# shendurelab/MIPGEN

Hardware: AMD Instinct MI355X
Metric: candidate MIPs scored/sec (SVR) (higher is better)
Workload: dtype f64

## Files before the change

mipgen_amd/csrc/accel_tiles.hip:

```cpp
#include "accel_internal.h"

extern "C" {

int mipgen_pick_sv_split(int n_tiles, int n_sv, int n_cu)
{
    const int groups = (n_sv + SVR_GROUP - 1) / SVR_GROUP;
    const double PH0 = 6.0;
    int best = 1;
    double best_cost = 0;
    for (int s = 1; s <= 8; s++) {
        if (s > 1 && groups / s < 32) break;
        const int64_t units = (int64_t)n_tiles * s, rounds = (units + n_cu - 1) / n_cu;
        const double cost = (double)rounds * (PH0 + (double)((groups + s - 1) / s));
        if (s == 1 || cost < best_cost * 0.98) { best = s; best_cost = cost; }
    }
    return best;
}

int mipgen_ensure_events(mipgen_accel* h)
{
    const size_t want = 4 * h->windows.size();
    while (h->ev.size() < want) {
        hipEvent_t e = nullptr;
        HIP_TRY(hipEventCreate(&e));
// ... 96 lines not shown
    auto shape_of = [&](const DevRegion& d, bool few) -> const Shape& {
        const int lanes = 64 * (few ? h->geom_few.wpc : h->geom.wpc);
        const uint64_t key = ((uint64_t)(uint32_t)d.n_pos << 32) | ((uint64_t)(uint16_t)d.k0 << 16) | (uint64_t)(uint16_t)d.n_sizes | (few ? (uint64_t)1 << 15 : 0);
        auto it = shapes.find(key);
        if (it != shapes.end()) return it->second;
        Shape best;
        double best_cost = 0;
        const int Cmax = D.max_capture - d.k0 * D.inc;
        for (int kc_cap = std::min(9, d.n_sizes); kc_cap >= 1; kc_cap--) {
            const int nkc = (d.n_sizes + kc_cap - 1) / kc_cap;
            if (kc_cap < std::min(9, d.n_sizes) && nkc == (d.n_sizes + kc_cap) / (kc_cap + 1)) continue;
            std::vector<Run> runs;
            double ent = 0, slots = 0;
            size_t lds_r = 0;
            bool ok = true;
            for (int c = 0; c < nkc && ok; c++) {
                const int ki0 = (int)((int64_t)d.n_sizes * c / nkc), ki1 = (int)((int64_t)d.n_sizes * (c + 1) / nkc);
                const int kc = ki1 - ki0;
                const int Cmax_t = Cmax - ki0 * D.inc, Cmin_t = Cmax_t - (kc - 1) * D.inc;
                const int ssmax = Cmax_t - D.min_sum, ssmin = Cmin_t - D.max_sum, ssr = ssmax - ssmin + 1;
                int np = std::max(1, std::min(lanes / kc, d.n_pos));
                size_t lds_t = 0;
                for (; np >= 1; np--) {
                    lds_t = mipgen_svr_lds_bytes_tile(np, ssr, ssmax, Lmax, n_arm, h->geom.group, h->geom.n_e, h->geom.n_l, h->geom.nchunk * h->geom.wpc * 64);
                    if (lds_t <= 160 * 1024) break;
                }
                if (np < 1) { ok = false; break; }
                { const int np_cf = np - ((np + D.inc) % 32); if (np_cf >= 1 && np_cf * 10 >= np * 9) { np = np_cf; lds_t = mipgen_svr_lds_bytes_tile(np, ssr, ssmax, Lmax, n_arm, h->geom.group, h->geom.n_e, h->geom.n_l, h->geom.nchunk * h->geom.wpc * 64); } }
                { const int nt = (d.n_pos + np - 1) / np, np_even = (d.n_pos + nt - 1) / nt;
                  if (np_even < np) { np = np_even; lds_t = mipgen_svr_lds_bytes_tile(np, ssr, ssmax, Lmax, n_arm, h->geom.group, h->geom.n_e, h->geom.n_l, h->geom.nchunk * h->geom.wpc * 64); } }
                runs.push_back({ki0, kc, np});
                lds_r = std::max(lds_r, lds_t);
                const double tiles = std::ceil((double)d.n_pos / np);
                ent += tiles * (np * (h->geom.n_e + h->geom.n_l) / 2.0 + (np + ssr - 1) * (h->geom.n_e + h->geom.n_l) / 2.0 + (double)np * ssr);
                slots += tiles * lanes;
            }
            if (!ok) continue;
            const double cost = 47.0 * ent + 2.7 * slots * D.n_pairs / 1.0;
            if (best.runs.empty() || cost < best_cost) { best.runs = runs; best_cost = cost; best.lds = lds_r; }
        }
        return shapes.emplace(key, std::move(best)).first->second;
    };
    for (Window& w : h->windows) {
        w.svr_tile0 = (int)st.size();
        int n_few_regions = 0;
        for (int i = w.r0; i < w.r1; i++) if (h->hregions[i].n_pos > 0 && h->hregions[i].n_sizes == 1) n_few_regions++;
        const bool win_few = h->have_few && n_few_regions >= h->n_cu;
        std::vector<uint8_t> st_few;
        for (int i = w.r0; i < w.r1; i++) {
            const DevRegion& d = h->hregions[i];
            if (d.n_pos <= 0 || d.n_sizes <= 0) continue;
            const bool few = win_few && d.n_sizes == 1;
            const Shape& shape = shape_of(d, false);
            if (shape.runs.empty()) { svr_lds = (size_t)1 << 30; continue; }
            svr_lds = std::max(svr_lds, shape.lds);
            const int Cmax = D.max_capture - d.k0 * D.inc;
            for (size_t lvl = 0; lvl < shape.runs.size(); lvl++) {
                const Run& r = shape.runs[lvl];
                max_levels = std::max(max_levels, (int)lvl + 1);
                for (int p0 = 0; p0 < d.n_pos; p0 += r.np) {
                    const int npt = std::min(r.np, d.n_pos - p0);
                    const int Cmax_t = Cmax - r.ki0 * D.inc, ssmax = Cmax_t - D.min_sum, ssr = (r.kc - 1) * D.inc + D.max_sum - D.min_sum + 1;
                    const double ent = (npt + (npt + ssr - 1)) * (h->geom.n_e + h->geom.n_l) / 2.0 + (double)npt * ssr;
                    const double cost = 19.0 * ent + 100.0 * (npt + ssmax + 2 * Lmax) + 75000.0;
                    const int fits = mipgen_svr_scores_fit_lds(npt, r.kc, D.n_pairs, ssr, ssmax, Lmax, n_arm, h->geom.group, h->geom.n_e, h->geom.n_l, h->geom.nchunk * h->geom.wpc * 64);
                    for (int s2 = 0; s2 < 2; s2++) { SvrTile t = {i, s2, p0, npt, r.ki0, r.kc, (int)lvl, fits}; st.push_back(t); st_cost.push_back(cost); st_few.push_back(few ? 1 : 0); }
                }
            }
        }
        {
            const size_t t0 = (size_t)w.svr_tile0, n = st.size() - t0;
            std::vector<size_t> order(n);
            for (size_t k = 0; k < n; k++) order[k] = k;
            std::stable_sort(order.begin(), order.end(), [&](size_t a, size_t b) { return st_few[a] != st_few[b] ? st_few[a] < st_few[b] : st_cost[t0 + a] > st_cost[t0 + b]; });
            std::vector<SvrTile> sorted(n);
            for (size_t k = 0; k < n; k++) sorted[k] = st[t0 + order[k]];
            std::copy(sorted.begin(), sorted.end(), st.begin() + (ptrdiff_t)t0);
            w.n_svr_few = 0;
            for (size_t k = 0; k < n; k++) w.n_svr_few += st_few[k];
        }
        w.n_svr_tiles = (int)st.size() - w.svr_tile0;
        {
            const size_t t0 = (size_t)w.svr_tile0, n = (size_t)w.n_svr_tiles;
            int wl = 0;
            for (size_t k = 0; k < n; k++) wl = std::max(wl, st[t0 + k].level + 1);
            w.lvl_tile0.assign(1, (int)st_lvl.size());
            for (int lvl = 0; lvl < wl; lvl++) {
                for (size_t k = 0; k < n; k++) if (st[t0 + k].level == lvl) st_lvl.push_back(st[t0 + k]);
                w.lvl_tile0.push_back((int)st_lvl.size());
// ... 35 lines not shown
```

mipgen_amd/csrc/common.h:

```cpp
#pragma once
#include <stdint.h>
#include "../../include/mipgen_accel.h"

#define BASE_A 0
#define BASE_C 1
#define BASE_G 2
#define BASE_T 3
#define BASE_N 4
#define BASE_DASH 5
#define BASE_OTHER 6
#define BASE_CODE_MASK 7
#define BASE_MASKED_BIT 8
#define BASE_SNP_SHIFT 4

#define F_EXT 0
#define F_EXT_GC 15
#define F_EXT_LEN 21
#define F_LRC 22
#define F_INS 66
#define F_INS_GC 129
#define F_INS_LEN 151
#define F_LIG 152
#define F_LIG_GC 167
#define F_LIG_LEN 173
// ... 91 lines not shown
    const int32_t* order;
};

struct SvrGeom {
    int32_t nchunk;
    int32_t chunk_len;
    int32_t n_e, n_l;
    int32_t group;
    int32_t wpc;
    int32_t pad[2];
};

#define SVR_MAX_CHUNK 15
#define SVR_GROUP 3
#define SVR_MAX_THREADS 1024
#define LOG_THREADS 256

#define SVR_N_ARR 7
struct SvrLayout {
    int rinv, lg10, rows, pf, tb, it;
    int ku, kd, ci, pf_stride;
    int tj, ti;
    int tu, td, tb_stride;
    int ssr_p;
    int bytes_kpar;
    int bytes_desc, bytes_ent, bytes_idx, bytes_sb, bytes_psum;
    int n_ent;
    int n_ent_lds;
    int total_bytes;
    int nq, ins_len, up_cnt, dn_cnt, span_b, rinv_len;
    int ins_sl, up_sl, dn_sl;
};

#if defined(__HIPCC__)
__host__ __device__
#endif
__attribute__((always_inline)) static inline int svr_arr_len(const SvrLayout& L, int k) { return k < 3 ? +L.ins_len : (k < 5 ? +L.up_cnt : +L.dn_cnt); }
#if defined(__HIPCC__)
__host__ __device__
#endif
__attribute__((always_inline)) static inline int svr_pad_slots(int len) { return (((len + 1 + 15) / 16) | 1) * 16; }
#if defined(__HIPCC__)
__host__ __device__
#endif
__attribute__((always_inline)) static inline int svr_arr_off(const SvrLayout& L, int k)
{
    const int ki = k < 3 ? k : 3, ku = k < 3 ? 0 : (k < 5 ? k - 3 : 2), kd = k < 5 ? 0 : k - 5;
    return ki * L.ins_sl + ku * L.up_sl + kd * L.dn_sl;
}
#if defined(__HIPCC__)
__host__ __device__
#endif
__attribute__((always_inline)) static inline int svr_arr_chunk(const SvrLayout& L, int k) { return (k < 3 ? +L.ins_sl : (k < 5 ? +L.up_sl : +L.dn_sl)) / 16; }
#if defined(__HIPCC__)
__host__ __device__
#endif
__attribute__((always_inline)) static inline SvrLayout svr_layout(int np, int ssmin, int ssmax, int Lmax, int n_arm, int group, int n_up, int n_dn, int n_threads)
{
    SvrLayout L;
    const int ssr = ssmax - ssmin + 1;
    L.nq = np + ssr - 1;
    L.ins_len = np + ssmax;
    L.up_cnt = Lmax + np;
    L.dn_cnt = L.nq + Lmax;
    L.ins_sl = svr_pad_slots(L.ins_len); L.up_sl = svr_pad_slots(L.up_cnt); L.dn_sl = svr_pad_slots(L.dn_cnt);
    L.span_b = np + ssmax + 2 * Lmax + 1;
    L.rinv_len = (ssmax > Lmax ? ssmax : Lmax) + 2;
    int o = 0;
    L.rinv = o; o += 3 * L.rinv_len;
    L.lg10 = o; o += 102 + 44;
    L.n_ent = np * n_up + L.nq * n_dn;
    L.rows = o; o += 2 * group * SV_ROW;
    int g = 3 * L.ins_sl + 2 * L.up_sl + 2 * L.dn_sl;
    L.ku = g; g += n_arm; L.kd = g; g += n_arm;
    L.ci = g; g += 1;
    L.tj = g; g += 18;
    L.ti = g; g += ssr;
    L.pf_stride = g;
    int pf_doubles = 2 * group * L.pf_stride;
    const int scratch_doubles = (np * (80 * 4 + ssr * 16) + 7) / 8;
    if (pf_doubles < scratch_doubles) pf_doubles = scratch_doubles;
    L.pf = o; o += pf_doubles;
    L.tu = 0; L.td = np * n_arm; L.tb_stride = np * n_arm + L.nq * n_arm;
    L.tb = o; o += group * L.tb_stride;
    L.ssr_p = ssr | 1;
    L.it = o; o += group * np * L.ssr_p;
    int bytes = o * 8;
    L.bytes_desc = bytes; bytes += SVR_N_ARR * 16 * 4;
    L.n_ent_lds = L.n_ent; (void)n_threads;
    L.bytes_ent = bytes; bytes += 2 * L.n_ent_lds * 4;
    L.bytes_psum = bytes; bytes += 2 * SVR_MAX_CHUNK * (SVR_MAX_THREADS / 64) + 16;
    bytes = (bytes + 15) & ~15;
    L.bytes_kpar = bytes; bytes += 64;
    L.bytes_idx = bytes;
    bytes += 4 * (3 * L.ins_sl + 2 * L.up_sl + 2 * L.dn_sl);
    L.bytes_sb = bytes; bytes += L.span_b + 8;
    L.total_bytes = (bytes + 15) & ~15;
    return L;
}
```

mipgen_amd/csrc/kernels.h:

```cpp
#pragma once
#include <hip/hip_runtime.h>
#include "common.h"
#include "reads_common.h"
#include "call_model.h"

struct HostConsts;
struct LrcMers { int8_t k[MIPGEN_N_LRC], code[MIPGEN_N_LRC], rc[MIPGEN_N_LRC]; };
struct FmtRegion {
    int32_t chr_off, chr_len;
    int32_t label_off, label_len;
    int32_t feature_start, feature_stop;
    int64_t rb0;
};
struct FmtConst {
    char middle[96];
    int32_t middle_len;
    int32_t n_regions;
    int64_t first_index;
};

struct KmerParams {
    int32_t n_k;
    int32_t k[MIPGEN_MAX_OLIGO];
    int32_t kmax;
// ... 17 lines not shown
    const uint2* __restrict__ units;
    int64_t n_small, n_big;
    const uint32_t* __restrict__ start;
    const int32_t* __restrict__ mol_len;
    const int64_t* __restrict__ pos_off;
    int32_t n;
    int64_t n_pos;
    uint32_t cell0;
    int min_family, min_quality;
};

struct CallCounters { unsigned long long tested, too_deep, candidates, calls; };
#define MIPGEN_CALL_MAX_POSITIONS (((int64_t)1 << 29) - 1)

struct LocusCounters { unsigned long long covered, bases, discordant, deletions, insertions, ins_discordant; };

extern "C" {
size_t mipgen_logistic_lds_bytes(int span);
hipError_t mipgen_launch_records_logistic(hipStream_t, int score, int n_tiles, int span_max, const DevParams*, const DevRegion*, const LogTile*, const uint8_t*, const int32_t*,
                                          const uint8_t*, const HostConsts*, double*, uint64_t*, int64_t* sat_idx, unsigned int* sat_count, unsigned int sat_cap);
size_t mipgen_logistic_dense_lds_bytes(int np_all, int np, int ssr, int ssmax, int Lmax, int n_up, int n_dn);
hipError_t mipgen_launch_logistic_dense(hipStream_t, int n_tiles, size_t lds_bytes, const DevParams*, const DevRegion*, const SvrTile*, const uint8_t*, const int32_t*,
                                        const uint8_t*, const HostConsts*, double*, uint64_t*, int64_t* sat_idx, unsigned int* sat_count, unsigned int sat_cap);
size_t mipgen_svr_lds_bytes_tile(int np, int ss_range, int ssmax, int Lmax, int n_arm, int group, int n_e, int n_l, int n_threads);
int mipgen_svr_scores_fit_lds(int np, int kc, int n_pairs, int ss_range, int ssmax, int Lmax, int n_arm, int group, int n_e, int n_l, int n_threads);
hipError_t mipgen_launch_svr_dense(hipStream_t, int n_tiles, int n_tiles_few, size_t lds_bytes, const DevParams*, const SvrGeom*, const SvrGeom* geom_few, const DevRegion*,
                                   const SvrTile*, const uint8_t*, const int32_t*, const double* log10_tab, const double* model, int n_sv, double gamma_l2e, double rho,
                                   double s_guard, const uint64_t* records, double* scores, int64_t n_cand, int n_split, double* partials);
hipError_t mipgen_launch_svr_run_state(hipStream_t s, int64_t n_pos, const DevParams* P, const DevRegion* regions, const int32_t* pos_region, const int32_t* pos_local,
                                       const uint32_t* run_bounds, int max_levels, int level, double margin, const double* scores, const uint64_t* records, double* pbs,
                                       uint8_t* state);
hipError_t mipgen_launch_svr_tile_keep(hipStream_t s, int n_tiles, const SvrTile* tiles, const int64_t* region_pos0, int64_t win_pos0, const uint8_t* state, int64_t* keep);
hipError_t mipgen_launch_svr_tile_compact(hipStream_t s, int n_tiles, const SvrTile* tiles, const int64_t* keep, const int64_t* offs, SvrTile* out, const DevParams* P,
                                          const DevRegion* regions, double* scores, unsigned long long* skipped);
hipError_t mipgen_launch_svr_gemm(hipStream_t, int n, const double* feats, const uint64_t* records, const double* model_t, const double* sv_norm, const double* sv_coef,
                                  const double* center, int n_sv_pad, double gamma, double rho, double* scores);
hipError_t mipgen_launch_dense_candidates(hipStream_t, const DevParams* P, const DevRegion* regions, int r0, int r1, int64_t c0, int n, mipgen_candidate* out);
hipError_t mipgen_launch_dense_list_fix(hipStream_t, int n, const uint64_t* records, double rho, double s_guard, double* scores);
hipError_t mipgen_launch_features_batch(hipStream_t, int n, const DevParams*, const DevRegion*, const mipgen_candidate*, const uint8_t* bases, const int32_t* copy,
                                        const uint8_t* unmap, const HostConsts*, uint64_t* records, double* features);
hipError_t mipgen_launch_candidates(hipStream_t, int n, const DevParams*, const DevRegion*, const mipgen_candidate*, const uint8_t*, const int32_t*, const uint8_t*,
                                    const HostConsts*, const double* model, int n_sv, double gamma, double rho, int method, double*, uint64_t*, double*, mipgen_candidate_ints*,
                                    int literal, const unsigned int* n_dev);
hipError_t mipgen_launch_candidates_probes(hipStream_t, int n, const ProbeSrc*, const HostConsts*, const double* model, int n_sv, double gamma, double rho, int method,
                                           double*, uint64_t*, double*, mipgen_candidate_ints*, int literal, const unsigned int* n_dev);
hipError_t mipgen_launch_probe_features(hipStream_t, int n, const ProbeSrc*, const HostConsts*, uint64_t* records, double* features);
hipError_t mipgen_launch_print_boundary_scan(hipStream_t, const DevParams*, const DevRegion*, const RescoreSrc*, double tol_rel, double tol_abs, mipgen_candidate* out,
                                             int64_t* out_idx, unsigned int* count, unsigned int cap, int n_cu);
// ... 82 lines not shown
```

mipgen_amd/csrc/kernels_svr.hip:

```cpp
#include <hip/hip_runtime.h>
#include "kernels.h"
#include "device_utils.h"
#include "exp2_coef.h"
#include "mip_record.h"
#include <stdlib.h>

namespace {

__device__ __forceinline__ void exp2x3(double& t0, double& t1, double& t2)
{
    constexpr double C[11] = EXP2_COEF_10;
    const double MAGIC = 6755399441055744.0;
    double m0, m1, m2, f0, f1, f2;
    const double cd = C[10];
    asm volatile(
        "v_add_f64 %[m0], %[t0], %[magic]\n\t"
        "v_add_f64 %[m1], %[t1], %[magic]\n\t"
        "v_add_f64 %[m2], %[t2], %[magic]\n\t"
        "v_add_f64 %[f0], %[m0], -%[magic]\n\t"
        "v_add_f64 %[f1], %[m1], -%[magic]\n\t"
        "v_add_f64 %[f2], %[m2], -%[magic]\n\t"
        "v_add_f64 %[f0], %[t0], -%[f0]\n\t"
        "v_add_f64 %[f1], %[t1], -%[f1]\n\t"
        "v_add_f64 %[f2], %[t2], -%[f2]\n\t"
// ... 33 lines not shown
          [c5] "s"(C[5]), [c6] "s"(C[6]), [c7] "s"(C[7]), [c8] "s"(C[8]), [c9] "s"(C[9]));
    t0 = __hiloint2double(__double2hiint(t0) + (__double2loint(m0) << 20), __double2loint(t0));
    t1 = __hiloint2double(__double2hiint(t1) + (__double2loint(m1) << 20), __double2loint(t1));
    t2 = __hiloint2double(__double2hiint(t2) + (__double2loint(m2) << 20), __double2loint(t2));
}

template <int N>
__device__ __forceinline__ double dpp_row_shr(double x)
{
    const int lo = __builtin_amdgcn_update_dpp(0, __double2loint(x), 0x110 | N, 0xf, 0xf, true);
    const int hi = __builtin_amdgcn_update_dpp(0, __double2hiint(x), 0x110 | N, 0xf, 0xf, true);
    return __hiloint2double(hi, lo);
}
__device__ __forceinline__ double readlane_f64(double x, int l)
{
    return __hiloint2double(__builtin_amdgcn_readlane(__double2hiint(x), l), __builtin_amdgcn_readlane(__double2loint(x), l));
}

__device__ __forceinline__ int arm_feat(int base, int idx) { return base + idx + (idx >= 15); }
__device__ __forceinline__ int ins_feat(int idx) { return F_INS + idx + (idx >= 63); }

}

extern "C" int mipgen_svr_scores_fit_lds(int np, int kc, int n_pairs, int ss_range, int ssmax, int Lmax, int n_arm, int group, int n_e, int n_l, int n_threads)
{
    const SvrLayout La = svr_layout(np, ssmax - ss_range + 1, ssmax, Lmax, n_arm, group, n_e, n_l, n_threads);
    const SvrLayout Lb = svr_layout(np, ssmax - ss_range + 1, ssmax, Lmax, n_arm, group, n_l, n_e, n_threads);
    const int need = np * kc * n_pairs;
    return need <= La.total_bytes / 8 - La.pf && need <= Lb.total_bytes / 8 - Lb.pf;
}

extern "C" size_t mipgen_svr_lds_bytes_tile(int np, int ss_range, int ssmax, int Lmax, int n_arm, int group, int n_e, int n_l, int n_threads)
{
    const SvrLayout La = svr_layout(np, ssmax - ss_range + 1, ssmax, Lmax, n_arm, group, n_e, n_l, n_threads);
    const SvrLayout Lb = svr_layout(np, ssmax - ss_range + 1, ssmax, Lmax, n_arm, group, n_l, n_e, n_threads);
    if ((size_t)La.tb_stride * group * 8 > 65535 || (size_t)Lb.tb_stride * group * 8 > 65535) return (size_t)1 << 30;
    const size_t a = (size_t)La.total_bytes, b = (size_t)Lb.total_bytes;
    return a > b ? a : b;
}

__device__ __forceinline__ void svr_steps2(double& a0, double& a1, uint32_t lu, uint32_t ld, uint32_t pg0, uint32_t pg1,
                                           double i00, double i01, double i02, double i10, double i11, double i12)
{
    double u00, u01, u02, d00, d01, d02, u10, u11, u12, d10, d11, d12;
    uint32_t au0, ad0, au1, ad1, s0, s1, s2, s3;
    asm volatile(
        "s_and_b32 %[s0], %[pg0], 0xffff\n\t"
        "s_lshr_b32 %[s1], %[pg0], 16\n\t"
        "s_and_b32 %[s2], %[pg1], 0xffff\n\t"
        "s_lshr_b32 %[s3], %[pg1], 16\n\t"
        "v_add_u32 %[au0], %[s0], %[lu]\n\t"
        "v_add_u32 %[ad0], %[s1], %[ld]\n\t"
        "v_add_u32 %[au1], %[s2], %[lu]\n\t"
        "v_add_u32 %[ad1], %[s3], %[ld]\n\t"
        "ds_read_b64 %[u00], %[au0]\n\t"
        "ds_read_b64 %[d00], %[ad0]\n\t"
        "ds_read_b64 %[u01], %[au0] offset:8\n\t"
        "ds_read_b64 %[d01], %[ad0] offset:8\n\t"
// ... 134 lines not shown
    const double* __restrict__ model = model_all + (int64_t)sv0 * SV_ROW;
    const int n_sv = max(0, min(n_sv_all - sv0, gpp * SVR_GROUP));
    const int tid = threadIdx.x, lane = tid & (WAVE - 1);
    const int wid = __builtin_amdgcn_readfirstlane(tid / WAVE);
    const int NT = blockDim.x, NW = NT / WAVE;
    const bool minus = tile.strand != 0;

    const int A = P->n_pairs;
    const int Lmax = max(P->e_max, P->l_max);
    const int n_arm = max(G.n_e, G.n_l) | 1;
    const int Cmax_t = P->max_capture - (R.k0 + tile.ki0) * P->inc;
    const int Cmin_t = Cmax_t - (tile.kc - 1) * P->inc;
    const int ssmax = Cmax_t - P->min_sum, ssmin = Cmin_t - P->max_sum;
    const int p_first = R.first_pos + tile.p0;
    const int lo = p_first - Lmax;
    const int up_min = minus ? +P->l_min : +P->e_min;
    const int dn_min = minus ? +P->e_min : +P->l_min;
    const int n_up = minus ? +G.n_l : +G.n_e, n_dn = minus ? +G.n_e : +G.n_l;
    const int up_base = minus ? F_LIG : F_EXT, dn_base = minus ? F_EXT : F_LIG;
    const int up_len_f = minus ? F_LIG_LEN : F_EXT_LEN, dn_len_f = minus ? F_EXT_LEN : F_LIG_LEN;
    const int up_cp_f = minus ? F_LLC : F_LEC, dn_cp_f = minus ? F_LEC : F_LLC;
    const int up_norm_f = minus ? SVR_N_LIG : SVR_N_EXT, dn_norm_f = minus ? SVR_N_EXT : SVR_N_LIG;

    const SvrLayout L = svr_layout(tile.np, ssmin, ssmax, Lmax, n_arm, SVR_GROUP, n_up, n_dn, (int)blockDim.x);
    int L_ku = L.ku, L_kd = L.kd, L_tu = L.tu, L_td = L.td, L_ins = L.ins_len, L_up = L.up_cnt, L_dn = L.dn_cnt;
    asm volatile("" : "+s"(L_ku), "+s"(L_kd), "+s"(L_tu), "+s"(L_td), "+s"(L_ins), "+s"(L_up), "+s"(L_dn));
    const int S_ins = __builtin_amdgcn_readfirstlane(L.ins_sl), S_up = __builtin_amdgcn_readfirstlane(L.up_sl), S_dn = __builtin_amdgcn_readfirstlane(L.dn_sl);
    double* const dbase = (double*)smem;
    double* rinv = dbase + L.rinv;
    double* lg10 = dbase + L.lg10;
    uint32_t* ent_a = (uint32_t*)(smem + L.bytes_ent);
    uint32_t* ent_b = ent_a + L.n_ent_lds;
    const double cneg = -gamma_l2e, c2 = 2.0 * gamma_l2e;
    uint16_t* psum = (uint16_t*)(smem + L.bytes_psum);
    uint32_t* work = (uint32_t*)(smem + L.bytes_psum + 2 * SVR_MAX_CHUNK * (SVR_MAX_THREADS / 64));
    double* rows = dbase + L.rows;
    double* pfb = dbase + L.pf;
    double* tbb = dbase + L.tb;
    double* itb = dbase + L.it;
    ScanDesc* desc = (ScanDesc*)(smem + L.bytes_desc);
    uint32_t* sidx = (uint32_t*)(smem + L.bytes_idx);
    uint8_t* sb = smem + L.bytes_sb;
    const int ssr = ssmax - ssmin + 1;
    const int nq_t = L.nq;

    for (int i = tid; i < L.span_b + 8; i += NT) {
        int ri = lo + i - R.seq_start;
        sb[i] = (i < L.span_b && ri >= 0 && ri < R.seq_len) ? (bases[R.seq_off + ri] & BASE_CODE_MASK) : (uint8_t)BASE_OTHER;
    }
    for (int i = tid; i < L.rinv_len; i += NT) {
        rinv[3 * i] = i > 0 ? 1.0 / (double)i : 0.0; rinv[3 * i + 1] = i > 1 ? 1.0 / (double)(i - 1) : 0.0;
        rinv[3 * i + 2] = i > 2 ? 1.0 / (double)(i - 2) : 0.0;
    }
    for (int i = tid; i < 102; i += NT) lg10[i] = i == 0 ? 0.0 : (i <= 100 ? log10_tab[i] : 2.0);
    for (int i = tid; i < MIPGEN_N_LRC; i += NT) lg10[102 + i] = R.lrc[i];
    for (int i = tid; i < A && i < SVR_MAX_CHUNK * (SVR_MAX_THREADS / 64); i += NT) psum[i] = (uint16_t)(P->arm_ext[i] + P->arm_lig[i]);
    if (tid < SVR_N_ARR) {
        ScanDesc d;
        const int k = tid;
        const bool ins = k < 3, up = k == 3 || k == 4;
        d.o0 = ins ? Lmax : (up ? 0 : Lmax + ssmin);
        d.k = ins ? k + 1 : ((k - 3) & 1) + 1;
        d.ax = ins ? 21 : 5; d.ay = ins ? 5 : 1; d.thr = ins ? 63 : 15;
        d.base = ins ? F_INS : (up ? up_base : dn_base);
        d.len = ins ? L_ins : (up ? L_up : L_dn);
        d.out = (ins ? k : 3) * S_ins + (ins ? 0 : (up ? k - 3 : 2)) * S_up + (k < 5 ? 0 : k - 5) * S_dn;
        d.ixo = d.out; d.c = (ins ? +S_ins : (up ? +S_up : +S_dn)) / 16;
        d.blk = ins ? 1 : ((up ? minus : !minus) ? 2 : 0);
        desc[k] = d;
    }
    __syncthreads();

    for (int k = 0; k < SVR_N_ARR; k++) {
        const ScanDesc d = desc[k];
        for (int i = tid; i < 16 * d.c; i += NT) {
            int slot = SVR_ZERO;
            if (i < d.len) {
                const int b0 = sb[d.o0 + i], b1 = sb[d.o0 + i + 1], b2 = sb[d.o0 + i + 2];
                const int last = d.k == 1 ? b0 : (d.k == 2 ? b1 : b2);
// ... 19 lines not shown
        (void)norm;
        int cp = 1;
        if (R.copy_off >= 0) {
            const int slot = P->len_slot[len];
            const int ri = lo + s - R.seq_start;
            cp = (slot >= 0 && ri >= 0 && ri < R.seq_len) ? copy[R.copy_off + (int64_t)slot * R.seq_len + ri] : 0;
        }
        const uint32_t cpc = (uint32_t)min(max(cp, 0), 101);
        uint32_t jcode = 0;
        if (is_lig) {
            int j0, j1;
            if (!minus) { j0 = sb[s]; j1 = sb[s + 1]; }
            else { j0 = comp_code(sb[s + len - 1]); j1 = comp_code(sb[s + len - 2]); }
            jcode = (j0 < 4 && j1 < 4) ? (uint32_t)(4 * j0 + j1 + 1) : 17u;
        }
        const int s0 = up ? s : wl;
        e_a = (uint32_t)((3 * S_ins + (up ? 0 : 2 * S_up) + s0) * (SVR_GROUP * 8)) | ((uint32_t)(((up ? L_tu : L_td) + wl * n_arm + li) * (SVR_GROUP * 8)) << 16);
        e_b = (uint32_t)len | ((uint32_t)up << 7) | ((jcode * (SVR_GROUP * 8)) << 8) | ((cpc * 8) << 17);
    };
    for (int w = tid; w < n_ent; w += NT) { uint32_t ea_, eb_; arm_entry(w, ea_, eb_, nullptr); ent_a[w] = ea_; ent_b[w] = eb_; }

    const int chunk = wid / G.wpc;
    const int item = (wid - chunk * G.wpc) * WAVE + lane;
    int np_lane = tile.np + (32 - (tile.np + P->inc) % 32) % 32;
    if (np_lane * tile.kc > G.wpc * WAVE) np_lane = tile.np;
    const int kci_l = item / np_lane, pl_l = item - kci_l * np_lane;
    const bool owner = chunk < G.nchunk && kci_l < tile.kc && pl_l < tile.np;
    const int kci = owner ? kci_l : 0, pl = owner ? pl_l : 0;
    const int a_lo = min(chunk, G.nchunk - 1) * G.chunk_len;
    const int a_n = min(G.chunk_len, A - a_lo);
    const int C = Cmax_t - kci * P->inc;
    const uint32_t lane_u_off = (uint32_t)((L.tu + pl * n_arm) * (SVR_GROUP * 8));
    const uint32_t lane_d_off = (uint32_t)((L.td + (pl + C - P->max_sum - ssmin) * n_arm) * (SVR_GROUP * 8));
    const int prog0 = __builtin_amdgcn_readfirstlane((minus ? MIPGEN_MAX_ARM_PAIRS + 16 : 0) + a_lo);
    uint32_t newS_v = 0;
#pragma unroll
    for (int i = 0; i < CL; i++) {
        const int a = a_lo + min(i, a_n - 1);
        if (i == 0 || (i < a_n && P->arm_ext[a - 1] + P->arm_lig[a - 1] != P->arm_ext[a] + P->arm_lig[a])) newS_v |= 1u << i;
    }
    const uint32_t newS = __builtin_amdgcn_readfirstlane(newS_v);
    const int iB = (pl * L.ssr_p + (C - ssmin)) * SVR_GROUP;
    double acc[CL];
#pragma unroll
    for (int i = 0; i < CL; i++) acc[i] = 0.0;
    const bool wave_owns = __builtin_amdgcn_ballot_w64(owner) != 0;

    if (tid == 0) {
        int* kp = (int*)(smem + L.bytes_kpar);
        kp[0] = nU; kp[1] = n_up; kp[2] = n_dn; kp[3] = up_min; kp[4] = dn_min; kp[5] = Lmax; kp[6] = ssmin; kp[7] = n_ent;
        kp[8] = L_tu; kp[9] = L_td; kp[10] = n_arm; kp[11] = tile.np; kp[12] = ssmax; kp[13] = L.ssr_p; kp[14] = minus ? 1 : 0;
    }

    const int n_groups = (n_sv + SVR_GROUP - 1) / SVR_GROUP;
    constexpr int ROW_N = SVR_GROUP * SV_ROW;
    constexpr int ROW_R = 1;
    const int64_t row_lim = (int64_t)n_sv * SV_ROW;
    auto row_fetch = [&](int k, int j) -> double {
        const int64_t gk = (int64_t)k * ROW_N + j;
        return (j < ROW_N && gk < row_lim) ? model[gk] : 0.0;
    };
    auto row_slot = [&](int k, int j) -> int { const int g = j / SV_ROW; return (k & 1) * ROW_N + (j - g * SV_ROW) * SVR_GROUP + g; };
    auto load_rows_direct = [&](int k) __attribute__((always_inline)) { for (int j = tid; j < ROW_N; j += NT) rows[row_slot(k, j)] = row_fetch(k, j); };

    typedef __attribute__((address_space(3))) const double lds_cd;
    typedef volatile __attribute__((address_space(3))) const double lds_vcd;
    typedef __attribute__((address_space(3))) double lds_d;
    typedef __attribute__((address_space(3))) const uint32_t lds_cu;
    constexpr int S_UNITS = 7;
    auto stage_scan = [&](int k) __attribute__((always_inline)) {
        lds_cd* rowk = (lds_cd*)rows + (k & 1) * ROW_N;
        lds_d* PF = (lds_d*)pfb + (k & 1) * SVR_GROUP * L.pf_stride;
        for (int u = wid; u < S_UNITS + 1; u += NW) {
            if (u < S_UNITS) {
// ... 137 lines not shown
                const uint32_t F1 = PF_a + __umul24((uint32_t)pi, SLOT);
                const uint32_t E1 = F1 + ss0 + ssiS;
                const uint32_t F2 = F1 + i1, F3 = F2 + i1;
                const uint32_t E2 = E1 + (i1 - SLOT), E3 = E1 + (2u * i1 - 2u * SLOT);
                const uint32_t Ti = PF_a + ti_off + ssiS;
                lds_vcd* rv = ldp(rv_a + __umul24((uint32_t)(ssmin + ssi), 24u));
                const double r0 = rv[0], r1 = rv[1], r2 = rv[2];
                lds_vcd* Cf = ldp(rowk_a + SVR_COEF * SLOT);
                double f1a[SVR_GROUP], f1b[SVR_GROUP], f2a[SVR_GROUP], f2b[SVR_GROUP], f3a[SVR_GROUP], f3b[SVR_GROUP], ti[SVR_GROUP], cf[SVR_GROUP];
#pragma unroll
                for (int g = 0; g < SVR_GROUP; g++) { f1a[g] = ldp(E1)[g]; f1b[g] = ldp(F1)[g]; f2a[g] = ldp(E2)[g]; f2b[g] = ldp(F2)[g]; f3a[g] = ldp(E3)[g]; f3b[g] = ldp(F3)[g]; ti[g] = ldp(Ti)[g]; cf[g] = Cf[g]; }
                __builtin_amdgcn_s_setprio(0);
#pragma unroll
                for (int g = 0; g < SVR_GROUP; g++) {
                    double t = ti[g];
                    t = fma(f1a[g] - f1b[g], r0, t);
                    t = fma(f2a[g] - f2b[g], r1, t);
                    t = fma(f3a[g] - f3b[g], r2, t);
                    x[g] = fmax(t, -330.0);
                }
                exp2x3(x[0], x[1], x[2]);
#pragma unroll
                for (int g = 0; g < SVR_GROUP; g++) x[g] *= cf[g];
                dst = it_a + __umul24((uint32_t)(__mul24(pi, L.ssr_p) + ssi), SLOT);
            }
            lds_d* dstp = (lds_d*)(unsigned long)dst;
#pragma unroll
            for (int g = 0; g < SVR_GROUP; g++) dstp[g] = x[g];
        }
    };

    load_rows_direct(0); load_rows_direct(1);
    if (tid == 0) *work = 0u;
    __syncthreads();
    if (!(dbg & 1)) stage_scan(0);
    __syncthreads();

    unsigned long long blk_t0 = 0; unsigned hwid = 0, xcc = 0;
    if ((dbg & 8) && prof) { blk_t0 = __builtin_amdgcn_s_memrealtime(); asm volatile("s_getreg_b32 %0, hwreg(HW_REG_HW_ID)" : "=s"(hwid)); asm volatile("s_getreg_b32 %0, hwreg(HW_REG_XCC_ID)" : "=s"(xcc)); }
    unsigned long long pc[6] = {0, 0, 0, 0, 0, 0};
    const bool stamp = (dbg & 8) && prof;
    typedef volatile __attribute__((address_space(3))) double lds_vd;
    const lds_vd* tb3 = (const lds_vd*)tbb;
    const lds_vd* it3 = (const lds_vd*)itb;
    const uint32_t tba = (uint32_t)(__UINTPTR_TYPE__)tb3;

    for (int i = 0; i < n_groups; i++) {
// ... 45 lines not shown
                } else {
                    svr_steps1(acc[ii], lane_u, lane_d, pg[ii], A0, A1, A2);
                }
            }
        }
        __builtin_amdgcn_s_setprio(0);
        const unsigned long long t4 = stamp ? __builtin_readcyclecounter() : 0;
#pragma unroll
        for (int r = 0; r < ROW_R; r++) { const int j = tid + r * NT; if (j < ROW_N) rows[row_slot(i, j)] = rowreg[r]; }
        for (int j = tid + ROW_R * NT; j < ROW_N; j += NT) rows[row_slot(i, j)] = row_fetch(i + 2, j);
        const unsigned long long t5 = stamp ? __builtin_readcyclecounter() : 0;
        __syncthreads();
        if (stamp) { const unsigned long long t6 = __builtin_readcyclecounter(); pc[0] += t1 - t0; pc[1] += t2 - t1; pc[2] += t4 - t3; pc[3] += t3 - t2; pc[4] += t6 - t0; pc[5] += t6 - t5; }
    }
    if (stamp && lane == 0 && blockIdx.x >= 400 && blockIdx.x < 432 && wid < 16) for (int k = 0; k < 6; k++) prof[((blockIdx.x - 400) * 16 + wid) * 6 + k] = pc[k];
    if (stamp && tid == 0 && blockIdx.x < 4096) { unsigned long long* q = prof + 64 * 8 * 6 + (size_t)blockIdx.x * 8; q[0] = hwid; q[1] = xcc; q[2] = blk_t0; q[3] = __builtin_amdgcn_s_memrealtime(); q[4] = blk_enter; q[6] = ((unsigned long long)tile.np << 32) | (unsigned)tile.kc; q[7] = ((unsigned long long)n_ent << 32) | (unsigned)(tile.np * ssr); }

    {
        volatile const int* kp = (volatile const int*)(smem + L.bytes_kpar);
        const int k_nU = __builtin_amdgcn_readfirstlane(kp[0]), k_nup = __builtin_amdgcn_readfirstlane(kp[1]), k_ndn = __builtin_amdgcn_readfirstlane(kp[2]);
        const int k_upmin = __builtin_amdgcn_readfirstlane(kp[3]), k_dnmin = __builtin_amdgcn_readfirstlane(kp[4]), k_Lmax = __builtin_amdgcn_readfirstlane(kp[5]);
        const int k_ssmin = __builtin_amdgcn_readfirstlane(kp[6]), k_nent = __builtin_amdgcn_readfirstlane(kp[7]), k_tu = __builtin_amdgcn_readfirstlane(kp[8]);
        const int k_td = __builtin_amdgcn_readfirstlane(kp[9]), k_narm = __builtin_amdgcn_readfirstlane(kp[10]), k_np = __builtin_amdgcn_readfirstlane(kp[11]);
        const int k_ssmax = __builtin_amdgcn_readfirstlane(kp[12]), k_ssrp = __builtin_amdgcn_readfirstlane(kp[13]), k_minus = __builtin_amdgcn_readfirstlane(kp[14]);
        const double kneg = -gamma_l2e;
        constexpr double CE[11] = EXP2_COEF_10;
        auto exp2_one = [&](double t) -> double {
            t = fmax(t, -1000.0);
            const double MAGIC = 6755399441055744.0;
            const double m = t + MAGIC;
            const double f = t - (m - MAGIC);
            double pp = CE[10];
#pragma unroll
            for (int k = 9; k >= 0; k--) pp = fma(pp, f, CE[k]);
            return __hiloint2double(__double2hiint(pp) + (__double2loint(m) << 20), __double2loint(pp));
        };
        uint32_t* cnt = (uint32_t*)pfb;
        int* insq = (int*)(cnt + 80 * k_np);
        const int k_ssr = k_ssmax - k_ssmin + 1;
        const int e1_waves = NW > 1 ? max(1, min((2 * k_np + WAVE - 1) / WAVE, NW / 2)) : 1;
        if (wid < e1_waves) {
            for (int pli = tid >> 1; pli < k_np; pli += e1_waves * (WAVE / 2)) {
                const int lvl = tid & 1;
                uint32_t* c = cnt + pli * 80 + (lvl ? 16 : 0);
                for (int k = 0; k < (lvl ? 64 : 16); k++) c[k] = 0;
                uint64_t c1p = 0;
                int q = 0, b1 = BASE_OTHER, b2 = BASE_OTHER;
// ... 39 lines not shown
                        }
                    }
                    prev = b;
                }
                int q2 = 0;
#pragma unroll
                for (int k = 0; k < 8; k++) {
                    const int a = (int)((clo >> (8 * k)) & 0xFF), b = (int)((chi >> (8 * k)) & 0xFF);
                    q2 += a * a + b * b;
                }
                const int c1[4] = {(int)(c1p & 0xFFFF), (int)((c1p >> 16) & 0xFFFF), (int)((c1p >> 32) & 0xFFFF), (int)(c1p >> 48)};
                const int q1 = c1[0] * c1[0] + c1[1] * c1[1] + c1[2] * c1[2] + c1[3] * c1[3];
                const double dl = (double)len, dl1 = (double)(len - 1);
                const double gc = (double)(c1[BASE_C] + c1[BASE_G]) / dl;
                tbb[((up ? k_tu : k_td) + wl * k_narm + li) * SVR_GROUP] = exp2_one(kneg * ((double)q1 / (dl * dl) + (double)q2 / (dl1 * dl1) + gc * gc));
            }
        }
        __syncthreads();
        for (int e = tid; e < k_np * k_ssr; e += NT) {
            const int pli = e / k_ssr, j = e - pli * k_ssr, n = k_ssmin + j;
            const int* o = insq + e * 4;
            const double dn = (double)n, dn1 = (double)(n - 1), dn2 = (double)(n - 2);
            const double gc = (double)o[2] / dn;
            itb[(pli * k_ssrp + j) * SVR_GROUP] = exp2_one(kneg * ((double)o[0] / (dn * dn) + (double)o[1] / (dn1 * dn1) + (double)o[3] / (dn2 * dn2) + gc * gc));
        }
        __syncthreads();
        if (owner) {
            const char* tbc = (const char*)tbb;
#pragma unroll
            for (int i = 0; i < CL; i++) {
                if (i < a_n) {
                    const uint32_t pgw = P->pair_prog[k_minus][a_lo + i];
                    const double fu = *(const double*)(tbc + lane_u_off + (pgw & 0xffffu)), fd = *(const double*)(tbc + lane_d_off + (pgw >> 16));
                    const double fi = itb[iB - (int)psum[a_lo + i] * SVR_GROUP];
                    acc[i] *= fu * fd * fi;
                }
            }
        }
    }

    {
        const int n_items = tile.np * tile.kc;
        const int nK = R.n_sizes;
        if (tile.pad) {
            double* const stg = dbase + L.pf;
            __syncthreads();
            if (owner) {
                const int item_own = kci * tile.np + pl;
#pragma unroll
                for (int i = 0; i < CL; i++) if (i < a_n) stg[item_own * A + a_lo + i] = acc[i];
            }
            __syncthreads();
            constexpr int WB = 4;
            for (int e0 = tid; e0 < n_items * A; e0 += WB * NT) {
                int64_t idx[WB];
                uint64_t rec[WB];
                double v[WB];
#pragma unroll
                for (int k = 0; k < WB; k++) {
                    const int e = min(e0 + k * NT, n_items * A - 1);
                    const int it_ = e / A, a = e - it_ * A;
                    const int kc_ = it_ / tile.np, pl_ = it_ - kc_ * tile.np;
                    idx[k] = R.out_off + ((((int64_t)(tile.p0 + pl_) * nK + (tile.ki0 + kc_)) * 2 + (minus ? 1 : 0)) * A) + a;
                    v[k] = stg[e];
                    rec[k] = n_split > 1 ? 0ull : records[idx[k]];
                }
#pragma unroll
// ... 102 lines not shown
```

Before: 1.799 billion.

## Transpose SVR insert-kernel table to size-major with bank-spreading pitch

Changes the insert kernel table in LDS from position-major with an odd size pitch to size-major with a per-tile pitch chosen so that lanes in a wave hit distinct LDS banks. The pitch is computed on the host, packed into the tile's pad field, and also used to pre-scale the psum offsets. Idle lanes are pointed at spread-out rows and columns rather than a shared one, so their dummy reads do not cause bank conflicts. The intent is fewer LDS bank conflicts in the hot accumulate loop, at the cost of a somewhat larger LDS footprint and extra host-side layout logic.

Result: faster. 1.823 billion, median of 6 (+1.4%).

```diff
diff --git a/mipgen_amd/csrc/accel_tiles.hip b/mipgen_amd/csrc/accel_tiles.hip
--- a/mipgen_amd/csrc/accel_tiles.hip
+++ b/mipgen_amd/csrc/accel_tiles.hip
@@ -142,13 +142,13 @@
                 int np = std::max(1, std::min(lanes / kc, d.n_pos));
                 size_t lds_t = 0;
                 for (; np >= 1; np--) {
-                    lds_t = mipgen_svr_lds_bytes_tile(np, ssr, ssmax, Lmax, n_arm, h->geom.group, h->geom.n_e, h->geom.n_l, h->geom.nchunk * h->geom.wpc * 64);
+                    lds_t = mipgen_svr_lds_bytes_tile(np, ssr, ssmax, Lmax, n_arm, h->geom.group, h->geom.n_e, h->geom.n_l, h->geom.nchunk * h->geom.wpc * 64, 0);
                     if (lds_t <= 160 * 1024) break;
                 }
                 if (np < 1) { ok = false; break; }
-                { const int np_cf = np - ((np + D.inc) % 32); if (np_cf >= 1 && np_cf * 10 >= np * 9) { np = np_cf; lds_t = mipgen_svr_lds_bytes_tile(np, ssr, ssmax, Lmax, n_arm, h->geom.group, h->geom.n_e, h->geom.n_l, h->geom.nchunk * h->geom.wpc * 64); } }
+                { const int np_cf = np - ((np + D.inc) % 32); if (np_cf >= 1 && np_cf * 10 >= np * 9) { np = np_cf; lds_t = mipgen_svr_lds_bytes_tile(np, ssr, ssmax, Lmax, n_arm, h->geom.group, h->geom.n_e, h->geom.n_l, h->geom.nchunk * h->geom.wpc * 64, 0); } }
                 { const int nt = (d.n_pos + np - 1) / np, np_even = (d.n_pos + nt - 1) / nt;
-                  if (np_even < np) { np = np_even; lds_t = mipgen_svr_lds_bytes_tile(np, ssr, ssmax, Lmax, n_arm, h->geom.group, h->geom.n_e, h->geom.n_l, h->geom.nchunk * h->geom.wpc * 64); } }
+                  if (np_even < np) { np = np_even; lds_t = mipgen_svr_lds_bytes_tile(np, ssr, ssmax, Lmax, n_arm, h->geom.group, h->geom.n_e, h->geom.n_l, h->geom.nchunk * h->geom.wpc * 64, 0); } }
                 runs.push_back({ki0, kc, np});
                 lds_r = std::max(lds_r, lds_t);
                 const double tiles = std::ceil((double)d.n_pos / np);
@@ -183,8 +183,11 @@
                     const int Cmax_t = Cmax - r.ki0 * D.inc, ssmax = Cmax_t - D.min_sum, ssr = (r.kc - 1) * D.inc + D.max_sum - D.min_sum + 1;
                     const double ent = (npt + (npt + ssr - 1)) * (h->geom.n_e + h->geom.n_l) / 2.0 + (double)npt * ssr;
                     const double cost = 19.0 * ent + 100.0 * (npt + ssmax + 2 * Lmax) + 75000.0;
-                    const int fits = mipgen_svr_scores_fit_lds(npt, r.kc, D.n_pairs, ssr, ssmax, Lmax, n_arm, h->geom.group, h->geom.n_e, h->geom.n_l, h->geom.nchunk * h->geom.wpc * 64);
-                    for (int s2 = 0; s2 < 2; s2++) { SvrTile t = {i, s2, p0, npt, r.ki0, r.kc, (int)lvl, fits}; st.push_back(t); st_cost.push_back(cost); st_few.push_back(few ? 1 : 0); }
+                    const int nthr = h->geom.nchunk * h->geom.wpc * 64;
+                    const int it_pitch = svr_it_pitch(npt, r.kc, D.inc, h->geom.wpc * 64, ssmax - ssr + 1, ssmax, Lmax, n_arm, h->geom.group, h->geom.n_e, h->geom.n_l, nthr);
+                    if (it_pitch) svr_lds = std::max(svr_lds, mipgen_svr_lds_bytes_tile(npt, ssr, ssmax, Lmax, n_arm, h->geom.group, h->geom.n_e, h->geom.n_l, nthr, it_pitch));
+                    const int fits = mipgen_svr_scores_fit_lds(npt, r.kc, D.n_pairs, ssr, ssmax, Lmax, n_arm, h->geom.group, h->geom.n_e, h->geom.n_l, nthr, it_pitch);
+                    for (int s2 = 0; s2 < 2; s2++) { SvrTile t = {i, s2, p0, npt, r.ki0, r.kc, (int)lvl, fits | (it_pitch << 8)}; st.push_back(t); st_cost.push_back(cost); st_few.push_back(few ? 1 : 0); }
                 }
             }
         }
diff --git a/mipgen_amd/csrc/common.h b/mipgen_amd/csrc/common.h
--- a/mipgen_amd/csrc/common.h
+++ b/mipgen_amd/csrc/common.h
@@ -137,7 +137,7 @@
     int ku, kd, ci, pf_stride;
     int tj, ti;
     int tu, td, tb_stride;
-    int ssr_p;
+    int it_p;
     int bytes_kpar;
     int bytes_desc, bytes_ent, bytes_idx, bytes_sb, bytes_psum;
     int n_ent;
@@ -170,7 +170,7 @@
 #if defined(__HIPCC__)
 __host__ __device__
 #endif
-__attribute__((always_inline)) static inline SvrLayout svr_layout(int np, int ssmin, int ssmax, int Lmax, int n_arm, int group, int n_up, int n_dn, int n_threads)
+__attribute__((always_inline)) static inline SvrLayout svr_layout(int np, int ssmin, int ssmax, int Lmax, int n_arm, int group, int n_up, int n_dn, int n_threads, int it_pitch)
 {
     SvrLayout L;
     const int ssr = ssmax - ssmin + 1;
@@ -198,8 +198,8 @@
     L.pf = o; o += pf_doubles;
     L.tu = 0; L.td = np * n_arm; L.tb_stride = np * n_arm + L.nq * n_arm;
     L.tb = o; o += group * L.tb_stride;
-    L.ssr_p = ssr | 1;
-    L.it = o; o += group * np * L.ssr_p;
+    L.it_p = it_pitch > 0 ? it_pitch : np;
+    L.it = o; o += group * (it_pitch > 0 ? ssr * it_pitch : np * (ssr | 1));
     int bytes = o * 8;
     L.bytes_desc = bytes; bytes += SVR_N_ARR * 16 * 4;
     L.n_ent_lds = L.n_ent; (void)n_threads;
@@ -213,3 +213,40 @@
     L.total_bytes = (bytes + 15) & ~15;
     return L;
 }
+
+#if defined(__HIPCC__)
+#define SVR_HD __host__ __device__ __attribute__((always_inline)) static inline
+#else
+#define SVR_HD __attribute__((always_inline)) static inline
+#endif
+#define SVR_LDS_LIMIT (160 * 1024)
+SVR_HD int svr_np_lane(int np, int kc, int inc, int lanes)
+{
+    const int padded = np + (32 - (np + inc) % 32) % 32;
+    return padded * kc > lanes ? np : padded;
+}
+SVR_HD bool svr_lane_pitch_spreads(int np_lane, int kc, int inc) { return kc == 1 || (np_lane + inc) % 32 == 0; }
+SVR_HD bool svr_it_pitch_spreads(int pitch, int np_lane, int kc, int inc)
+{
+    return (pitch & 1) && (kc == 1 || (((np_lane + inc * pitch) % 32) + 32) % 32 == 0);
+}
+SVR_HD int svr_idle_d_row(int j, int np_lane, int kc, int inc, int nq, int sum_span)
+{
+    const int r = (j + (kc - 1) * inc) & 31;
+    return svr_lane_pitch_spreads(np_lane, kc, inc) && r + sum_span < nq ? r : (kc - 1) * inc;
+}
+SVR_HD int svr_idle_it_col(int j, int pitch, int np_lane, int kc, int inc)
+{
+    return svr_it_pitch_spreads(pitch, np_lane, kc, inc) && (j & 31) < pitch ? (j & 31) : 0;
+}
+static inline int svr_it_pitch(int np, int kc, int inc, int lanes, int ssmin, int ssmax, int Lmax, int n_arm, int group, int n_e, int n_l, int n_threads)
+{
+    const int np_lane = svr_np_lane(np, kc, inc, lanes);
+    auto fits = [&](int pitch) {
+        return svr_layout(np, ssmin, ssmax, Lmax, n_arm, group, n_e, n_l, n_threads, pitch).total_bytes <= SVR_LDS_LIMIT &&
+               svr_layout(np, ssmin, ssmax, Lmax, n_arm, group, n_l, n_e, n_threads, pitch).total_bytes <= SVR_LDS_LIMIT;
+    };
+    for (int pitch = np; pitch < np + 64; pitch++)
+        if (svr_it_pitch_spreads(pitch, np_lane, kc, inc)) { if (fits(pitch)) return pitch; break; }
+    return fits(np | 1) ? (np | 1) : 0;
+}
diff --git a/mipgen_amd/csrc/kernels.h b/mipgen_amd/csrc/kernels.h
--- a/mipgen_amd/csrc/kernels.h
+++ b/mipgen_amd/csrc/kernels.h
@@ -63,8 +63,8 @@
 size_t mipgen_logistic_dense_lds_bytes(int np_all, int np, int ssr, int ssmax, int Lmax, int n_up, int n_dn);
 hipError_t mipgen_launch_logistic_dense(hipStream_t, int n_tiles, size_t lds_bytes, const DevParams*, const DevRegion*, const SvrTile*, const uint8_t*, const int32_t*,
                                         const uint8_t*, const HostConsts*, double*, uint64_t*, int64_t* sat_idx, unsigned int* sat_count, unsigned int sat_cap);
-size_t mipgen_svr_lds_bytes_tile(int np, int ss_range, int ssmax, int Lmax, int n_arm, int group, int n_e, int n_l, int n_threads);
-int mipgen_svr_scores_fit_lds(int np, int kc, int n_pairs, int ss_range, int ssmax, int Lmax, int n_arm, int group, int n_e, int n_l, int n_threads);
+size_t mipgen_svr_lds_bytes_tile(int np, int ss_range, int ssmax, int Lmax, int n_arm, int group, int n_e, int n_l, int n_threads, int it_pitch);
+int mipgen_svr_scores_fit_lds(int np, int kc, int n_pairs, int ss_range, int ssmax, int Lmax, int n_arm, int group, int n_e, int n_l, int n_threads, int it_pitch);
 hipError_t mipgen_launch_svr_dense(hipStream_t, int n_tiles, int n_tiles_few, size_t lds_bytes, const DevParams*, const SvrGeom*, const SvrGeom* geom_few, const DevRegion*,
                                    const SvrTile*, const uint8_t*, const int32_t*, const double* log10_tab, const double* model, int n_sv, double gamma_l2e, double rho,
                                    double s_guard, const uint64_t* records, double* scores, int64_t n_cand, int n_split, double* partials);
diff --git a/mipgen_amd/csrc/kernels_svr.hip b/mipgen_amd/csrc/kernels_svr.hip
--- a/mipgen_amd/csrc/kernels_svr.hip
+++ b/mipgen_amd/csrc/kernels_svr.hip
@@ -79,18 +79,18 @@
 
 }
 
-extern "C" int mipgen_svr_scores_fit_lds(int np, int kc, int n_pairs, int ss_range, int ssmax, int Lmax, int n_arm, int group, int n_e, int n_l, int n_threads)
-{
-    const SvrLayout La = svr_layout(np, ssmax - ss_range + 1, ssmax, Lmax, n_arm, group, n_e, n_l, n_threads);
-    const SvrLayout Lb = svr_layout(np, ssmax - ss_range + 1, ssmax, Lmax, n_arm, group, n_l, n_e, n_threads);
+extern "C" int mipgen_svr_scores_fit_lds(int np, int kc, int n_pairs, int ss_range, int ssmax, int Lmax, int n_arm, int group, int n_e, int n_l, int n_threads, int it_pitch)
+{
+    const SvrLayout La = svr_layout(np, ssmax - ss_range + 1, ssmax, Lmax, n_arm, group, n_e, n_l, n_threads, it_pitch);
+    const SvrLayout Lb = svr_layout(np, ssmax - ss_range + 1, ssmax, Lmax, n_arm, group, n_l, n_e, n_threads, it_pitch);
     const int need = np * kc * n_pairs;
     return need <= La.total_bytes / 8 - La.pf && need <= Lb.total_bytes / 8 - Lb.pf;
 }
 
-extern "C" size_t mipgen_svr_lds_bytes_tile(int np, int ss_range, int ssmax, int Lmax, int n_arm, int group, int n_e, int n_l, int n_threads)
-{
-    const SvrLayout La = svr_layout(np, ssmax - ss_range + 1, ssmax, Lmax, n_arm, group, n_e, n_l, n_threads);
-    const SvrLayout Lb = svr_layout(np, ssmax - ss_range + 1, ssmax, Lmax, n_arm, group, n_l, n_e, n_threads);
+extern "C" size_t mipgen_svr_lds_bytes_tile(int np, int ss_range, int ssmax, int Lmax, int n_arm, int group, int n_e, int n_l, int n_threads, int it_pitch)
+{
+    const SvrLayout La = svr_layout(np, ssmax - ss_range + 1, ssmax, Lmax, n_arm, group, n_e, n_l, n_threads, it_pitch);
+    const SvrLayout Lb = svr_layout(np, ssmax - ss_range + 1, ssmax, Lmax, n_arm, group, n_l, n_e, n_threads, it_pitch);
     if ((size_t)La.tb_stride * group * 8 > 65535 || (size_t)Lb.tb_stride * group * 8 > 65535) return (size_t)1 << 30;
     const size_t a = (size_t)La.total_bytes, b = (size_t)Lb.total_bytes;
     return a > b ? a : b;
@@ -271,7 +271,7 @@
     const int up_cp_f = minus ? F_LLC : F_LEC, dn_cp_f = minus ? F_LEC : F_LLC;
     const int up_norm_f = minus ? SVR_N_LIG : SVR_N_EXT, dn_norm_f = minus ? SVR_N_EXT : SVR_N_LIG;
 
-    const SvrLayout L = svr_layout(tile.np, ssmin, ssmax, Lmax, n_arm, SVR_GROUP, n_up, n_dn, (int)blockDim.x);
+    const SvrLayout L = svr_layout(tile.np, ssmin, ssmax, Lmax, n_arm, SVR_GROUP, n_up, n_dn, (int)blockDim.x, tile.pad >> 8);
     int L_ku = L.ku, L_kd = L.kd, L_tu = L.tu, L_td = L.td, L_ins = L.ins_len, L_up = L.up_cnt, L_dn = L.dn_cnt;
     asm volatile("" : "+s"(L_ku), "+s"(L_kd), "+s"(L_tu), "+s"(L_td), "+s"(L_ins), "+s"(L_up), "+s"(L_dn));
     const int S_ins = __builtin_amdgcn_readfirstlane(L.ins_sl), S_up = __builtin_amdgcn_readfirstlane(L.up_sl), S_dn = __builtin_amdgcn_readfirstlane(L.dn_sl);
@@ -303,7 +303,7 @@
     }
     for (int i = tid; i < 102; i += NT) lg10[i] = i == 0 ? 0.0 : (i <= 100 ? log10_tab[i] : 2.0);
     for (int i = tid; i < MIPGEN_N_LRC; i += NT) lg10[102 + i] = R.lrc[i];
-    for (int i = tid; i < A && i < SVR_MAX_CHUNK * (SVR_MAX_THREADS / 64); i += NT) psum[i] = (uint16_t)(P->arm_ext[i] + P->arm_lig[i]);
+    for (int i = tid; i < A && i < SVR_MAX_CHUNK * (SVR_MAX_THREADS / 64); i += NT) psum[i] = (uint16_t)((P->arm_ext[i] + P->arm_lig[i]) * L.it_p);
     if (tid < SVR_N_ARR) {
         ScanDesc d;
         const int k = tid;
@@ -369,8 +369,7 @@
 
     const int chunk = wid / G.wpc;
     const int item = (wid - chunk * G.wpc) * WAVE + lane;
-    int np_lane = tile.np + (32 - (tile.np + P->inc) % 32) % 32;
-    if (np_lane * tile.kc > G.wpc * WAVE) np_lane = tile.np;
+    const int np_lane = svr_np_lane(tile.np, tile.kc, P->inc, G.wpc * WAVE);
     const int kci_l = item / np_lane, pl_l = item - kci_l * np_lane;
     const bool owner = chunk < G.nchunk && kci_l < tile.kc && pl_l < tile.np;
     const int kci = owner ? kci_l : 0, pl = owner ? pl_l : 0;
@@ -378,7 +377,8 @@
     const int a_n = min(G.chunk_len, A - a_lo);
     const int C = Cmax_t - kci * P->inc;
     const uint32_t lane_u_off = (uint32_t)((L.tu + pl * n_arm) * (SVR_GROUP * 8));
-    const uint32_t lane_d_off = (uint32_t)((L.td + (pl + C - P->max_sum - ssmin) * n_arm) * (SVR_GROUP * 8));
+    const int d_row = owner ? pl + C - P->max_sum - ssmin : svr_idle_d_row(item, np_lane, tile.kc, P->inc, nq_t, P->max_sum - P->min_sum);
+    const uint32_t lane_d_off = (uint32_t)((L.td + d_row * n_arm) * (SVR_GROUP * 8));
     const int prog0 = __builtin_amdgcn_readfirstlane((minus ? MIPGEN_MAX_ARM_PAIRS + 16 : 0) + a_lo);
     uint32_t newS_v = 0;
 #pragma unroll
@@ -387,7 +387,8 @@
         if (i == 0 || (i < a_n && P->arm_ext[a - 1] + P->arm_lig[a - 1] != P->arm_ext[a] + P->arm_lig[a])) newS_v |= 1u << i;
     }
     const uint32_t newS = __builtin_amdgcn_readfirstlane(newS_v);
-    const int iB = (pl * L.ssr_p + (C - ssmin)) * SVR_GROUP;
+    const int it_pl = owner ? pl : svr_idle_it_col(item, L.it_p, np_lane, tile.kc, P->inc);
+    const int iB = ((C - ssmin) * L.it_p + it_pl) * SVR_GROUP;
     double acc[CL];
 #pragma unroll
     for (int i = 0; i < CL; i++) acc[i] = 0.0;
@@ -396,7 +397,7 @@
     if (tid == 0) {
         int* kp = (int*)(smem + L.bytes_kpar);
         kp[0] = nU; kp[1] = n_up; kp[2] = n_dn; kp[3] = up_min; kp[4] = dn_min; kp[5] = Lmax; kp[6] = ssmin; kp[7] = n_ent;
-        kp[8] = L_tu; kp[9] = L_td; kp[10] = n_arm; kp[11] = tile.np; kp[12] = ssmax; kp[13] = L.ssr_p; kp[14] = minus ? 1 : 0;
+        kp[8] = L_tu; kp[9] = L_td; kp[10] = n_arm; kp[11] = tile.np; kp[12] = ssmax; kp[13] = L.it_p; kp[14] = minus ? 1 : 0;
     }
 
     const int n_groups = (n_sv + SVR_GROUP - 1) / SVR_GROUP;
@@ -580,7 +581,7 @@
                 exp2x3(x[0], x[1], x[2]);
 #pragma unroll
                 for (int g = 0; g < SVR_GROUP; g++) x[g] *= cf[g];
-                dst = it_a + __umul24((uint32_t)(__mul24(pi, L.ssr_p) + ssi), SLOT);
+                dst = it_a + __umul24((uint32_t)(__mul24(ssi, L.it_p) + pi), SLOT);
             }
             lds_d* dstp = (lds_d*)(unsigned long)dst;
 #pragma unroll
@@ -672,7 +673,7 @@
         const int k_upmin = __builtin_amdgcn_readfirstlane(kp[3]), k_dnmin = __builtin_amdgcn_readfirstlane(kp[4]), k_Lmax = __builtin_amdgcn_readfirstlane(kp[5]);
         const int k_ssmin = __builtin_amdgcn_readfirstlane(kp[6]), k_nent = __builtin_amdgcn_readfirstlane(kp[7]), k_tu = __builtin_amdgcn_readfirstlane(kp[8]);
         const int k_td = __builtin_amdgcn_readfirstlane(kp[9]), k_narm = __builtin_amdgcn_readfirstlane(kp[10]), k_np = __builtin_amdgcn_readfirstlane(kp[11]);
-        const int k_ssmax = __builtin_amdgcn_readfirstlane(kp[12]), k_ssrp = __builtin_amdgcn_readfirstlane(kp[13]), k_minus = __builtin_amdgcn_readfirstlane(kp[14]);
+        const int k_ssmax = __builtin_amdgcn_readfirstlane(kp[12]), k_itp = __builtin_amdgcn_readfirstlane(kp[13]), k_minus = __builtin_amdgcn_readfirstlane(kp[14]);
         const double kneg = -gamma_l2e;
         constexpr double CE[11] = EXP2_COEF_10;
         auto exp2_one = [&](double t) -> double {
@@ -758,7 +759,7 @@
             const int* o = insq + e * 4;
             const double dn = (double)n, dn1 = (double)(n - 1), dn2 = (double)(n - 2);
             const double gc = (double)o[2] / dn;
-            itb[(pli * k_ssrp + j) * SVR_GROUP] = exp2_one(kneg * ((double)o[0] / (dn * dn) + (double)o[1] / (dn1 * dn1) + (double)o[3] / (dn2 * dn2) + gc * gc));
+            itb[(j * k_itp + pli) * SVR_GROUP] = exp2_one(kneg * ((double)o[0] / (dn * dn) + (double)o[1] / (dn1 * dn1) + (double)o[3] / (dn2 * dn2) + gc * gc));
         }
         __syncthreads();
         if (owner) {
@@ -778,7 +779,7 @@
     {
         const int n_items = tile.np * tile.kc;
         const int nK = R.n_sizes;
-        if (tile.pad) {
+        if (tile.pad & 1) {
             double* const stg = dbase + L.pf;
             __syncthreads();
             if (owner) {
```
